# TMmichi/mujoco_jaco

Hardware: AMD Instinct MI355X
Metric: env-steps/sec at batch 65 536 (full Jaco + gripper + contacts) (higher is better)
Workload: dtype f32

## Files before the change

### mujoco_jaco_amd/csrc/collision.h

```cpp
#pragma once

#define JACO_HAVE_COLLISION 1

struct GeomPose { v3 p; m3 R; };
template <class L>
JDEV GeomPose geom_pose(const L& s, int g) { GeomPose r; r.p = ld3(s.gpos[g]); r.R = ldm(s.gmat[g]); return r; }

JDEV bool obb_separated(const GeomPose& a, v3 sa, const GeomPose& b, v3 sb) {
  float C[3][3], Q[3][3];
  v3 d = b.p - a.p;
  float t[3] = {dot(d, col(a.R, 0)), dot(d, col(a.R, 1)), dot(d, col(a.R, 2))};
  float ea[3] = {sa.x, sa.y, sa.z}, eb[3] = {sb.x, sb.y, sb.z};
#pragma unroll
  for (int i = 0; i < 3; i++)
#pragma unroll
    for (int j = 0; j < 3; j++) { C[i][j] = dot(col(a.R, i), col(b.R, j)); Q[i][j] = fabsf(C[i][j]) + 1e-5f; }
  bool sep = false;
#pragma unroll
  for (int i = 0; i < 3; i++) sep |= fabsf(t[i]) > ea[i] + eb[0] * Q[i][0] + eb[1] * Q[i][1] + eb[2] * Q[i][2];
#pragma unroll
  for (int j = 0; j < 3; j++)
    sep |= fabsf(t[0] * C[0][j] + t[1] * C[1][j] + t[2] * C[2][j]) > eb[j] + ea[0] * Q[0][j] + ea[1] * Q[1][j] + ea[2] * Q[2][j];
#pragma unroll
  for (int i = 0; i < 3; i++)
// ... 36 lines not shown
JDEV v3 support_geom(const JacoStepArgs& A, const JacoModelDev* m, const L& s, int g, int type, v3 dir, int lane) {
  GeomPose P = geom_pose(s, g);
  v3 l = mulT(P.R, dir), sp;
  if (type == JG_BOX) {
    sp = mk3(l.x > 0.f ? m->g_size[g][0] : -m->g_size[g][0], l.y > 0.f ? m->g_size[g][1] : -m->g_size[g][1], l.z > 0.f ? m->g_size[g][2] : -m->g_size[g][2]);
  } else if (type == JG_SPHERE) {
    float n = norm(l);
    sp = l * (n > JMINVAL ? m->g_size[g][0] / n : 0.f);
  } else {
    int adr = m->g_vertadr[g], nvert = m->g_vertnum[g];
    float best = -3.0e38f;
    int bi = 0x7fffffff;
    for (int i = lane; i < nvert; i += 64) {
      const float* v = A.hull + 4 * (size_t)(adr + i);
      float t = v[0] * l.x + v[1] * l.y + v[2] * l.z;
      if (t > best) { best = t; bi = i; }
    }
    float bv;
    int win = wave_argmax(best, bi, &bv);
    win = win < nvert ? win : 0;
    const float* v = A.hull + 4 * (size_t)(adr + win);
    sp = mk3(v[0], v[1], v[2]);
  }
  return P.p + mul(P.R, sp);
}

template <class L>
JDEV void collide_plane_box(v3 size, L& s, int g1, int g2, int pair, int lane, int& ncon, unsigned& flags) {
  GeomPose P = geom_pose(s, g1), B = geom_pose(s, g2);
  v3 n = col(P.R, 2);
  int i = lane & 7;
  v3 l = mk3((i & 1) ? size.x : -size.x, (i & 2) ? size.y : -size.y, (i & 4) ? size.z : -size.z);
  v3 c = B.p + mul(B.R, l);
  float dist = dot(c - P.p, n);
  push_contacts(s, lane < 8 && !(dist > 0.f), dist, c - n * (0.5f * dist), n, pair, ncon, flags, 4);
}
template <class L>
JDEV void collide_plane_sphere(const JacoModelDev* m, L& s, int g1, int g2, int pair, int lane, int& ncon, unsigned& flags) {
  GeomPose P = geom_pose(s, g1);
  v3 n = col(P.R, 2), c = ld3(s.gpos[g2]);
  float r = m->g_size[g2][0], dist = dot(c - P.p, n) - r;
  push_contacts(s, lane == 0 && !(dist > 0.f), dist, c - n * (r + 0.5f * dist), n, pair, ncon, flags, 1);
}
template <class L>
JDEV void collide_plane_convex(const JacoStepArgs& A, const JacoModelDev* m, L& s, int g1, int g2, int t2, int pair, int lane, int& ncon, unsigned& flags) {
  GeomPose P = geom_pose(s, g1);
  v3 n = col(P.R, 2);
  v3 sp = support_geom(A, m, s, g2, t2, -n, lane);
  float dist = dot(sp - P.p, n);
  push_contacts(s, lane == 0 && !(dist > 0.f), dist, sp - n * (0.5f * dist), n, pair, ncon, flags, 1);
}

template <class L>
JDEV void collide_box_box4(const JacoModelDev* m, L& s, int cbase, int nrows, int pkA, int codeA, unsigned m1A, unsigned m2A, int obA, int dimA,
                           v3 saA, v3 sbA, int lane, int& ncon, unsigned& flags) {
  constexpr int MAXCON = L::Caps::MAXCON;
  const int g = lane >> 4, a = lane & 15, rb = lane & 48;
  const bool slot = g < nrows;
  const int src = cbase + (slot ? g : 0);
  const int code = wave_shfl_i(codeA, src), pair = wave_shfl_i(pkA, src);
  const unsigned pm1 = (unsigned)wave_shfl_i((int)m1A, src), pm2 = (unsigned)wave_shfl_i((int)m2A, src);
  const int pob = wave_shfl_i(obA, src), pdim = wave_shfl_i(dimA, src);
  const int g1 = code & 255, g2 = (code >> 8) & 255;
  GeomPose P1 = geom_pose(s, g1), P2 = geom_pose(s, g2);
  float s1[3] = {wave_shfl(saA.x, src), wave_shfl(saA.y, src), wave_shfl(saA.z, src)}, s2[3] = {wave_shfl(sbA.x, src), wave_shfl(sbA.y, src), wave_shfl(sbA.z, src)};
  (void)m;
  v3 Aa[3] = {col(P1.R, 0), col(P1.R, 1), col(P1.R, 2)}, Ba[3] = {col(P2.R, 0), col(P2.R, 1), col(P2.R, 2)};
  v3 pp = P2.p - P1.p;
  const int ai = a < 15 ? a : 0;
  int ei = ai >= 6 ? (ai - 6) / 3 : (ai < 3 ? ai : 0), ej = ai >= 6 ? (ai - 6) % 3 : (ai >= 3 ? ai - 3 : 0);
  v3 Ai = ei == 0 ? Aa[0] : (ei == 1 ? Aa[1] : Aa[2]), Bj = ej == 0 ? Ba[0] : (ej == 1 ? Ba[1] : Ba[2]);
  v3 ax = ai < 3 ? Ai : (ai < 6 ? Bj : cross(Ai, Bj));
  float len = norm(ax);
  bool degenerate = ai >= 6 && len < 1e-6f;
  ax = ax * (1.f / fmaxf(len, 1e-30f));
  float ra = s1[0] * fabsf(dot(ax, Aa[0])) + s1[1] * fabsf(dot(ax, Aa[1])) + s1[2] * fabsf(dot(ax, Aa[2]));
  float rb_ = s2[0] * fabsf(dot(ax, Ba[0])) + s2[1] * fabsf(dot(ax, Ba[1])) + s2[2] * fabsf(dot(ax, Ba[2]));
  float dp = dot(pp, ax), pen = ra + rb_ - fabsf(dp);
  bool mine = slot && a < 15 && !degenerate;
  const unsigned long long sepm = wave_ballot(mine && pen < 0.f);
  const bool alive = slot && ((sepm >> rb) & 0xffffull) == 0ull;
  if (wave_ballot(alive) == 0ull) return;
  float fbest, ebest;
  int fcode = row_argmax(a < 6 ? -pen : -3.0e38f, a, &fbest);
  int ecode = row_argmax((a >= 6 && mine) ? -pen : -3.0e38f, a, &ebest);
  fbest = -fbest; ebest = -ebest;
  const bool edge = ebest < 1.0e38f && ebest * 1.05f < fbest;
  bool h1 = false, h2 = false;
  float d1 = 0.f, d2 = 0.f;
  v3 x1 = mk3(0, 0, 0), x2 = mk3(0, 0, 0), nrm = mk3(0, 0, 1.f);
  if (wave_ballot(alive && edge)) {
    const int ec = edge ? ecode : 6;
    const int i = (ec - 6) / 3, j = (ec - 6) % 3;
    float sgn = wave_shfl(dp, rb + ec) < 0.f ? -1.f : 1.f;
    v3 n = mk3(wave_shfl(ax.x, rb + ec), wave_shfl(ax.y, rb + ec), wave_shfl(ax.z, rb + ec)) * sgn;
    v3 ea = P1.p, eb = P2.p;
#pragma unroll
    for (int k = 0; k < 3; k++) {
      const v3 ea2 = ea + Aa[k] * (dot(n, Aa[k]) > 0.f ? s1[k] : -s1[k]), eb2 = eb + Ba[k] * (dot(n, Ba[k]) > 0.f ? -s2[k] : s2[k]);
      if (k != i) ea = ea2;
      if (k != j) eb = eb2;
    }
    v3 ua = i == 0 ? Aa[0] : (i == 1 ? Aa[1] : Aa[2]), ub = j == 0 ? Ba[0] : (j == 1 ? Ba[1] : Ba[2]);
    v3 r = eb - ea;
    float uv = dot(ua, ub), du = dot(r, ua), dv = dot(r, ub), den = 1.f - uv * uv;
    float sa = den > 1e-12f ? (du - uv * dv) / den : 0.f, tb = den > 1e-12f ? (uv * du - dv) / den : 0.f;
    if (alive && edge) {
      h1 = a == 0; d1 = -ebest; nrm = n;
      x1 = ((ea + ua * sa) + (eb + ub * tb)) * 0.5f;
    }
  }
  if (wave_ballot(alive && !edge)) {
    bool refis1 = fcode < 3;
    int ia = refis1 ? fcode : fcode - 3;
// ... 34 lines not shown
      const float kx = (k == 1 || k == 2) ? 1.f : -1.f, ky = k >= 2 ? 1.f : -1.f;
      const v3 q0 = c2 + eu * kx + ev * ky;
      if (a < 4) {
        hv1 = fabsf(q0.x) <= a_ && fabsf(q0.y) <= b_;
        pt1 = q0;
      } else if (a < 8) {
        float det = eu.x * ev.y - eu.y * ev.x;
        if (fabsf(det) > 1e-14f) {
          float x = kx * a_ - c2.x, y = ky * b_ - c2.y;
          float al = (x * ev.y - y * ev.x) / det, be = (eu.x * y - eu.y * x) / det;
          hv1 = fabsf(al) < 1.f && fabsf(be) < 1.f;
          pt1 = mk3(kx * a_, ky * b_, c2.z + al * eu.z + be * ev.z);
        }
      }
    }
    {
      const int k = a >> 2, k1 = (k + 1) & 3;
      const float kx = (k == 1 || k == 2) ? 1.f : -1.f, ky = k >= 2 ? 1.f : -1.f;
      const float k1x = (k1 == 1 || k1 == 2) ? 1.f : -1.f, k1y = k1 >= 2 ? 1.f : -1.f;
      const v3 q0 = c2 + eu * kx + ev * ky, q1 = c2 + eu * k1x + ev * k1y;
      const int e = a & 3, axn = e & 1;
      float lim = ((e & 2) ? 1.f : -1.f) * (axn ? b_ : a_), other = axn ? a_ : b_;
      float q0a = axn ? q0.y : q0.x, q1a = axn ? q1.y : q1.x, q0o = axn ? q0.x : q0.y, q1o = axn ? q1.x : q1.y;
      float e0 = q0a - lim, e1 = q1a - lim;
      if (!((e0 < 0.f) == (e1 < 0.f) || e0 == e1)) {
        float t = e0 / (e0 - e1);
        float o = q0o + t * (q1o - q0o);
        if (t > 0.f && t < 1.f && fabsf(o) < other) {
          hv2 = true;
          pt2 = axn ? mk3(o, lim, q0.z + t * (q1.z - q0.z)) : mk3(lim, o, q0.z + t * (q1.z - q0.z));
        }
      }
    }
    if (alive && !edge) {
      h1 = hv1 && !(pt1.z > 0.f); h2 = hv2 && !(pt2.z > 0.f);
      d1 = 0.5f * pt1.z; d2 = 0.5f * pt2.z;
      x1 = rp + Ru * pt1.x + Rv * pt1.y + nref * (rn + 0.5f * pt1.z);
      x2 = rp + Ru * pt2.x + Rv * pt2.y + nref * (rn + 0.5f * pt2.z);
      nrm = nref * (refis1 ? 1.f : -1.f);
    }
  }
  const unsigned long long M1 = wave_ballot(h1), M2 = wave_ballot(h2);
  int off = 0, tot = 0;
#pragma unroll
  for (int r = 0; r < 4; r++) {
    const int cr = popc64((M1 >> (16 * r)) & 0xffffull) + popc64((M2 >> (16 * r)) & 0xffffull);
    off += r < g ? cr : 0;
    tot += cr;
  }
  const unsigned long long r1 = (M1 >> rb) & 0xffffull, r2 = (M2 >> rb) & 0xffffull, below = (1ull << a) - 1ull;
  const int i1 = ncon + off + popc64(r1 & below), i2 = ncon + off + popc64(r1) + popc64(r2 & below);
  if (h1 && i1 < MAXCON) {
    s.c_dist[i1] = d1; st3(s.c_pos[i1], x1); make_frame(nrm, s.c_frame[i1]); s.c_pair[i1] = pair;
    s.c_m1[i1] = pm1; s.c_m2[i1] = pm2; s.c_ob[i1] = pob; s.c_dim[i1] = pdim;
  }
  if (h2 && i2 < MAXCON) {
    s.c_dist[i2] = d2; st3(s.c_pos[i2], x2); make_frame(nrm, s.c_frame[i2]); s.c_pair[i2] = pair;
    s.c_m1[i2] = pm1; s.c_m2[i2] = pm2; s.c_ob[i2] = pob; s.c_dim[i2] = pdim;
  }
  if (ncon + tot > MAXCON) { flags |= JFLAG_CON_OVERFLOW; tot = MAXCON - ncon; }
  ncon += tot;
}

struct Sup { v3 v, v1; };
struct MprGeom { GeomPose P; v3 size; int type, adr, nvert, cellR, celladr; };
#ifdef JACO_ROW_REUSE
struct HullRow { int cell; v4 e; };
#define JROWARG , HullRow& H1, HullRow& H2
#define JROWPASS , H1, H2
#else
#define JROWARG
#define JROWPASS
#endif
template <class L>
JDEV MprGeom mpr_geom(const JacoModelDev* m, const L& s, int g, int type) {
  MprGeom G;
  G.P = geom_pose(s, g);
  G.size = ld3(m->g_size[g]);
  G.type = type;
  G.adr = type == JG_MESH ? m->g_vertadr[g] : 0;
  G.nvert = type == JG_MESH ? m->g_vertnum[g] : 0;
  G.cellR = type == JG_MESH ? m->g_cellR[g] : 0;
  G.celladr = type == JG_MESH ? m->g_celladr[g] : 0;
  return G;
}
JDEV int cube_cell(v3 d, int R) {
  float ax = fabsf(d.x), ay = fabsf(d.y), az = fabsf(d.z);
  const bool fx = ax >= ay && ax >= az, fy = !fx && ay >= az;
  int face = fx ? (d.x > 0.f ? 0 : 1) : (fy ? (d.y > 0.f ? 2 : 3) : (d.z > 0.f ? 4 : 5));
  float mx = fx ? ax : (fy ? ay : az);
  mx = mx < 1e-30f ? 1.f : mx;
  float u = (fx ? d.y : d.x) / mx, v = ((fx || fy) ? d.z : d.y) / mx;
  int iu = (int)floorf((u + 1.f) * 0.5f * (float)R), iv = (int)floorf((v + 1.f) * 0.5f * (float)R);
  iu = iu < 0 ? 0 : (iu > R - 1 ? R - 1 : iu);
  iv = iv < 0 ? 0 : (iv > R - 1 ? R - 1 : iv);
  return (face * R + iu) * R + iv;
}
JDEV v3 support_prim(const MprGeom& G, v3 l) {
  if (G.type == JG_BOX) return mk3(l.x > 0.f ? G.size.x : -G.size.x, l.y > 0.f ? G.size.y : -G.size.y, l.z > 0.f ? G.size.z : -G.size.z);
  if (G.type == JG_CYLINDER) {
    const float rr = sqrtf(l.x * l.x + l.y * l.y), k = rr > JMINVAL ? G.size.x / rr : 0.f;
    return mk3(l.x * k, l.y * k, l.z > 0.f ? G.size.y : -G.size.y);
  }
  float n = norm(l);
  return l * (n > JMINVAL ? G.size.x / n : 0.f);
}
JDEV Sup mpr_support(const JacoStepArgs& A, const MprGeom& G1, const MprGeom& G2, v3 dir, int lane JROWARG) {
#ifdef JACO_EMULATED
  if (lane == 0) emu_counter[7]++;
#endif
  const v3 l1 = mulT(G1.P.R, dir), l2 = mulT(G2.P.R, -dir);
// ... 468 lines not shown
    for (int G = 0; 256 * G < npair; G++) {
      if (4 * G < plane_chunks) sphere_group<true>(s, m, G, npair, lane, n1, nl, tmp, PL::NV * 64); else sphere_group<false>(s, m, G, npair, lane, n1, nl, tmp, PL::NV * 64);
    }
#endif
    wave_sync();
    pl.n = nl <= PL::NV * 64 ? nl : -1;
    pl.planes = 0u;
#pragma unroll
    for (int j = 0; j < PL::NV; j++) {
      const bool have = j * 64 + lane < nl && pl.n >= 0;
      pl.e[j] = have ? tmp[have ? j * 64 + lane : 0] : 0u;
      pl.planes |= wave_ballot(have && ((pl.e[j] >> (JPL_KBITS + 2 * JPL_GBITS)) & 1u) != 0u) ? 1u << j : 0u;
    }
#pragma unroll
    for (int p = 0; p < JGEOM_PASSES; p++) { pl.px[p] = gp[p].x; pl.py[p] = gp[p].y; pl.pz[p] = gp[p].z; }
  } else {
#pragma unroll
    for (int j = 0; j < PL::NV; j++) {
      if (j * 64 < pl.n) {
        const bool valid = j * 64 + lane < pl.n;
        if ((pl.planes >> j) & 1u) list_chunk<true>(s, pl.e[j], valid, n1); else list_chunk<false>(s, pl.e[j], valid, n1);
      }
    }
  }
  JSTAMP(9);
  if (lane == 0) s.nsphere = n1;
  if (n1 > L::Caps::MAXCAND) { flags |= JFLAG_CAND_OVERFLOW; n1 = L::Caps::MAXCAND; }
  wave_sync();
  int ncand = 0;
  for (int base = 0; base < n1; base += 64) {
    int ci = base + lane;
    int k = ci < n1 ? s.cand[ci] : 0;
    bool keep = ci < n1;
    if (keep) {
      const v4 q0 = ld4(reinterpret_cast<const float*>(&m->pair_obb[k])), q1 = ld4(reinterpret_cast<const float*>(&m->pair_obb[k]) + 4);
      const int code = __builtin_bit_cast(int, q0.x);
      int g1 = code & 255, g2 = (code >> 8) & 255, t1 = (code >> 16) & 15;
      if (t1 != JG_PLANE) keep = !obb_separated(geom_pose(s, g1), mk3(q0.y, q0.z, q0.w), geom_pose(s, g2), mk3(q1.x, q1.y, q1.z));
    }
    wave_sync();
    unsigned long long mask = wave_ballot(keep);
    if (keep) s.cand[ncand + wave_prefix_count(mask)] = k;
    ncand += popc64(mask);
    wave_sync();
  }
  JSTAMP(10);
  int ncon = 0;
  for (int cb = 0; cb < ncand; cb += 64) {
    const int nhere = ncand - cb < 64 ? ncand - cb : 64;
    const int pkA = s.cand[lane < nhere ? cb + lane : cb];
    const v4 rec0 = ld4(reinterpret_cast<const float*>(&m->pair_obb[pkA])), rec1 = ld4(reinterpret_cast<const float*>(&m->pair_obb[pkA]) + 4);
    const int codeA = __builtin_bit_cast(int, rec0.x);
    const v3 saA = mk3(rec0.y, rec0.z, rec0.w), sbA = mk3(rec1.x, rec1.y, rec1.z);
    const unsigned m1A = m->pair[pkA].m1, m2A = m->pair[pkA].m2;
    const int obA = m->pair[pkA].ob, dimA = m->pair[pkA].condim;
    const unsigned long long boxes = wave_ballot(lane < nhere && ((codeA >> 16) & 255) == (JG_BOX | (JG_BOX << 4)));
    const unsigned long long hullc = wave_ballot(lane < nhere && ((codeA >> 16) & 15) != JG_PLANE && ((codeA >> 16) & 255) != (JG_BOX | (JG_BOX << 4)));
    v4 sepA; sepA.x = sepA.y = sepA.z = sepA.w = 0.f;
    float* const seprow = A.sepdir ? A.sepdir + (size_t)env * (4 * JMAXPAIR) : nullptr;
    if (seprow && lane < nhere && ((codeA >> 16) & 15) != JG_PLANE && ((codeA >> 16) & 255) != (JG_BOX | (JG_BOX << 4))) sepA = ld4(seprow + 4 * pkA);
    JSTAMP_NARROW(11);
#if JACO_MPR_PAIRS
    float* const stash = s.early_scratch;
    static_assert(JSCRATCH >= 512, "MPR result stash");
    unsigned long long parked = 0ull;
    if (A.mpr_pairs && popc64(hullc) >= 2) {
      const int gA1 = codeA & 255, gA2 = (codeA >> 8) & 255;
      const bool okA = lane < nhere && !((((codeA >> 16) & 15) == JG_MESH && m->g_cellR[gA1] == 0) || (((codeA >> 20) & 15) == JG_MESH && m->g_cellR[gA2] == 0));
      unsigned long long todo = hullc & wave_ballot(okA);
      while (popc64(todo) >= 2) {
        lane = wave_opaque_i(lane);
        const int c1 = ffs64(todo); todo &= todo - 1ull;
        const int c2 = ffs64(todo); todo &= todo - 1ull;
        const int cc = lane < 32 ? c1 : c2;
        const int pk2 = wave_shfl_i(pkA, cc), code2 = wave_shfl_i(codeA, cc);
        const MprGeom H1 = mpr_geom(m, s, code2 & 255, (code2 >> 16) & 15), H2 = mpr_geom(m, s, (code2 >> 8) & 255, (code2 >> 20) & 15);
        v4 sd; sd.x = wave_shfl(sepA.x, cc); sd.y = wave_shfl(sepA.y, cc); sd.z = wave_shfl(sepA.z, cc); sd.w = wave_shfl(sepA.w, cc);
        bool hit2, sv2, ran2;
        float depth2;
        v3 dir2, pos2, sep2;
        mpr_pair2(A, m, H1, H2, sd, true, lane, &hit2, &depth2, &dir2, &pos2, &sep2, &sv2, &ran2);
        if ((lane & 31) == 0) {
          if (seprow && ran2 && (sv2 || sd.w != 0.f)) {
            v4 o; o.x = sep2.x; o.y = sep2.y; o.z = sep2.z; o.w = sv2 ? 1.f : 0.f;
            *reinterpret_cast<v4*>(seprow + 4 * pk2) = o;
          }
          float* st = stash + 8 * cc;
          st[0] = hit2 ? 1.f : 0.f; st[1] = depth2; st[2] = pos2.x; st[3] = pos2.y; st[4] = pos2.z; st[5] = dir2.x; st[6] = dir2.y; st[7] = dir2.z;
#ifdef JACO_EMULATED
          emu_counter[3]++; emu_counter[4] += hit2;
#endif
        }
#ifdef JACO_EMULATED
        if (lane == 0) emu_counter[10]++;
#endif
        parked |= (1ull << c1) | (1ull << c2);
      }
      wave_sync();
      JSTAMP_NARROW(14);
    }
#else
    const unsigned long long parked = 0ull;
    (void)hullc;
#endif
    for (int c = 0; c < nhere;) {
      lane = wave_opaque_i(lane);
      if (L::Caps::MAXEFC < JacoHuge::MAXEFC && (wave_uniform_i((int)flags) & (int)JFLAG_CON_OVERFLOW)) break;
      if ((boxes >> c) & 1ull) {
        const int run = ffs64(~(boxes >> c) | 16ull);
        collide_box_box4(m, s, c, run, pkA, codeA, m1A, m2A, obA, dimA, saA, sbA, lane, ncon, flags);
        c += run;
        JSTAMP_NARROW(12);
        continue;
      }
      const int pk = wave_bcast_i(pkA, c), code = wave_bcast_i(codeA, c);
      const unsigned pm1 = (unsigned)wave_bcast_i((int)m1A, c), pm2 = (unsigned)wave_bcast_i((int)m2A, c);
      const int pob = wave_bcast_i(obA, c), pdim = wave_bcast_i(dimA, c);
      const int g1 = code & 255, g2 = (code >> 8) & 255, t1 = (code >> 16) & 15, t2 = (code >> 20) & 15;
      const int before = ncon;
      if (t1 == JG_PLANE) {
        if (t2 == JG_BOX) collide_plane_box(mk3(wave_bcast(sbA.x, c), wave_bcast(sbA.y, c), wave_bcast(sbA.z, c)), s, g1, g2, pk, lane, ncon, flags);
        else if (t2 == JG_SPHERE) collide_plane_sphere(m, s, g1, g2, pk, lane, ncon, flags);
        else if (t2 == JG_MESH) collide_plane_convex(A, m, s, g1, g2, t2, pk, lane, ncon, flags);
        JSTAMP_NARROW(13);
      } else {
        float depth;
        v3 dir, pos;
#ifdef JACO_EMULATED
        const long q0_ = emu_counter[7];
#endif
        const MprGeom G1 = mpr_geom(m, s, g1, t1), G2 = mpr_geom(m, s, g2, t2);
#ifdef JACO_ROW_REUSE
        HullRow H1, H2;
        H1.cell = -1; H2.cell = -1; H1.e.x = H1.e.y = H1.e.z = H1.e.w = 0.f; H2.e = H1.e;
#endif
        const float sw = wave_bcast(sepA.w, c);
        bool hit = false, apart = false, sepvalid = false;
        v3 sep = mk3(0.f, 0.f, 0.f);
#if JACO_MPR_PAIRS
        if ((parked >> c) & 1ull) {
          const float* st = stash + 8 * c;
          hit = st[0] != 0.f; depth = st[1]; pos = mk3(st[2], st[3], st[4]); dir = mk3(st[5], st[6], st[7]);
          apart = true;
        } else
#endif
        if (sw != 0.f) {
          const v3 d = mk3(wave_bcast(sepA.x, c), wave_bcast(sepA.y, c), wave_bcast(sepA.z, c));
          const Sup q = mpr_support(A, G1, G2, d, lane JROWPASS);
          apart = dot(q.v, d) < -1e-5f && fabsf(dot(d, d) - 1.f) < 1e-3f;
        }
        if (!apart) {
          hit = mpr_penetration(A, m, G1, G2, lane, &depth, &dir, &pos, &sep, &sepvalid JROWPASS);
          if (seprow && lane == 0 && (sepvalid || sw != 0.f)) {
            v4 o; o.x = sep.x; o.y = sep.y; o.z = sep.z; o.w = sepvalid ? 1.f : 0.f;
            *reinterpret_cast<v4*>(seprow + 4 * pk) = o;
          }
        }
#ifdef JACO_EMULATED
        if (lane == 0 && !((parked >> c) & 1ull)) { emu_counter[3]++; emu_counter[4] += hit; emu_counter[hit ? 5 : 6] += emu_counter[7] - q0_; }
#endif
#ifdef JACO_TRACE_MPR
        if (lane == 0) printf("mpr g1 %d g2 %d hit %d depth %g\n", g1, g2, (int)hit, hit ? depth : 0.f);
#endif
        push_contacts(s, hit && lane == 0, -depth, pos, dir, pk, ncon, flags, 1);
        JSTAMP_NARROW(hit ? 14 : 1);
      }
      if (ncon > before) {
        int cc = before + lane;
        if (cc < ncon) { s.c_m1[cc] = pm1; s.c_m2[cc] = pm2; s.c_ob[cc] = pob; s.c_dim[cc] = pdim; }
      }
      c++;
    }
    if (L::Caps::MAXEFC < JacoHuge::MAXEFC && (wave_uniform_i((int)flags) & (int)JFLAG_CON_OVERFLOW)) break;
  }
  if (lane == 0) { s.ncon = ncon; s.ncand = ncand; }
}

#define JSIDE_ROWS 16
#define JSIDE_BASE 64
#define JSIDE_J 0
#define JSIDE_AREF 96
#define JSIDE_D 112
#define JSIDE_F 128
template <class L>
struct SideRows {
  static constexpr bool on = L::Caps::CONTACT && L::Caps::MAXEFC == 64 && JNV - JB1 == 6 && (JNV - 6) * 6 + JNB * 6 >= JSIDE_F + JSIDE_ROWS;
};
template <class L>
JDEV float* side_buf(L& s) { return &s.cdof[6][0]; }
template <class L>
JDEV float contact_row_vel(const L& s, int c, int e, float mu) {
  const int pd = s.c_dim[c];
  const int kf = pd == 1 ? 0 : 1 + (e >> 1);
  const int obs = s.c_ob[c], b1 = ((obs >> 8) & 0xFF) - 1, b2 = ((obs >> 24) & 0xFF) - 1;
  sv v1, v2;
  v1.a = v1.b = v2.a = v2.b = mk3(0.f, 0.f, 0.f);
  if (b1 >= 0) v1 = ldsv(s.cvel[b1]);
  if (b2 >= 0) v2 = ldsv(s.cvel[b2]);
  v3 cp = ld3(s.c_pos[c]);
  v3 dw = v2.a - v1.a, dv = (v2.b - v1.b) + cross(dw, cp);
  const float* fr = s.c_frame[c];
  float vel = dot(ld3(fr), dv);
  if (pd > 1) {
    const int ax = kf < 3 ? kf : kf - 3;
    const float comp = dot(ld3(fr + 3 * ax), kf < 3 ? dv : dw);
    vel += ((e & 1) ? -1.f : 1.f) * mu * comp;
  }
  return vel;
}
template <class L>
JDEV void stage_contact_rows(const JacoModelDev* m, L& s, int lane, unsigned& flags) {
  constexpr int MAXEFC = L::Caps::MAXEFC;
  constexpr bool SIDE = SideRows<L>::on;
  const int nv = m->nv, ncon = wave_uniform_i(s.ncon), nlim = wave_uniform_i(s.nlimit);
  float* pa0 = reinterpret_cast<float*>(s.c_m1);
  float* pbc = reinterpret_cast<float*>(s.c_m2);
  float* sd = side_buf(s);
  int rowbase = nlim, kept_total = 0, nside = 0, side_cand = 0;
  constexpr int CPP = JNV <= 21 ? 3 : 64 / JNV;
  const int cl = lane / JNV, k = lane - cl * JNV;
  const bool dofok = cl < CPP && k < nv;
  const sv S = ldsv(s.cdof[dofok ? k : 0]);
  for (int cb = 0; cb < ncon; cb += 64) {
    const int ci = cb + lane, nhere = ncon - cb < 64 ? ncon - cb : 64;
    int dim = 0, nrow = 0;
    float mu0 = 0.f, mu1 = 0.f, mu2 = 0.f;
    unsigned cm1 = 0, cm2 = 0;
    float a0 = 0.f, bcoef = 0.f, dinv = 0.f;
    if (lane < nhere) {
      const JacoPairParam& P = m->pair[s.c_pair[ci]];
      dim = s.c_dim[ci]; nrow = dim == 1 ? 1 : 2 * (dim - 1);
      mu0 = P.mu[0]; mu1 = P.mu[2]; mu2 = P.mu[3];
      cm1 = s.c_m1[ci]; cm2 = s.c_m2[ci];
      const float pos = s.c_dist[ci] - P.margin, tran = P.tran;
      float R, imp;
      a0 = row_params(P.solref, P.solimp, pos, 0.f, dim == 1 ? tran : tran + mu0 * mu0 * tran, &R, &imp);
      bcoef = 2.f / fmaxf(JMINVAL, fminf(0.9999f, fmaxf(0.0001f, P.solimp[1])) * P.solref[0]);
      if (dim > 1) R = fmaxf(JMINVAL, 2.f * mu0 * mu0 * R);
      dinv = 1.f / R;
    }
    const unsigned mm = cm1 | cm2;
    bool sidec = false;
    const unsigned long long upto = lane >= 63 ? ~0ull : ((2ull << lane) - 1ull);
    const unsigned long long r1m = wave_ballot(nrow == 1), r4m = wave_ballot(nrow == 4), r10m = wave_ballot(nrow == 10);
    const bool rows_std = wave_ballot(nrow != 0 && nrow != 1 && nrow != 4 && nrow != 10) == 0ull;
    int end = rowbase + (rows_std ? popc64(r1m & upto) + 4 * popc64(r4m & upto) + 10 * popc64(r10m & upto) : wave_scan_incl(nrow, lane));
#ifdef JACO_SIDE_ALWAYS
    if (JNV - JB1 == 6 && cb == 0) {
#else
    if (JNV - JB1 == 6 && cb == 0 && wave_bcast_i(end, nhere - 1) > JSIDE_BASE) {
#endif
      const bool only2 = lane < nhere && mm != 0u && (mm & ((1u << JB1) - 1u)) == 0u && nrow <= 4;
      const bool reach2 = lane < nhere && !only2 && (mm >> JB1) != 0u;
      const unsigned long long o2 = wave_ballot(only2);
      if (o2 != 0ull && wave_ballot(reach2) == 0ull && ncon <= 64) {
        int srows = 0;
        for (unsigned long long b = o2; b; b &= b - 1ull) srows += wave_bcast_i(nrow, ffs64(b));
        if (srows <= JSIDE_ROWS) { side_cand = srows; sidec = only2; }
      }
    }
    bool split = false;
    int r0s = 0;
#ifdef JACO_SIDE_ALWAYS
    if (SIDE && side_cand > 0 && wave_bcast_i(end, nhere - 1) - side_cand <= MAXEFC) {
#else
    if (SIDE && side_cand > 0 && wave_bcast_i(end, nhere - 1) > MAXEFC && wave_bcast_i(end, nhere - 1) - side_cand <= MAXEFC) {
#endif
      split = true;
      end = rowbase + wave_scan_incl(sidec ? 0 : nrow, lane);
      r0s = JSIDE_BASE + wave_scan_incl(sidec ? nrow : 0, lane) - nrow;
      nside = side_cand;
    }
    sidec = sidec && split;
    const unsigned long long fm = wave_ballot(lane < nhere && end <= MAXEFC);
    const int kept = popc64(fm);
    int total = wave_bcast_i(end, kept > 0 ? kept - 1 : 0);
    total = kept > 0 ? total : rowbase;
    const int r0 = sidec ? r0s : end - nrow;
    if (lane < kept) {
      s.c_efc[ci] = r0;
      int blk = ((mm & ((1u << JB0) - 1u)) ? 1 : 0) | (((mm >> JB0) & ((1u << (JB1 - JB0)) - 1u)) ? 2 : 0) | ((mm >> JB1) ? 4 : 0);
      const int bodies = L::Caps::WRENCH ? ((((s.c_ob[ci] >> 8) & 31) << 19) | (((s.c_ob[ci] >> 24) & 31) << 24)) : 0;
      if (!sidec) for (int e = 0; e < nrow; e++) {
        s.e_con[r0 + e] = ci | (e << 8) | (blk << 16) | bodies;
        s.e_f[r0 + e] = e < 4 ? mu0 : (e < 6 ? mu1 : mu2);
      }
      pa0[ci] = a0; pbc[ci] = bcoef; s.c_fn[ci] = dinv;
    }
    wave_sync();
    for (int rr = rowbase + lane; rr < total; rr += 64) {
      const int ce = s.e_con[rr], c = ce & 255, e = (ce >> 8) & 255;
      const float vel = contact_row_vel(s, c, e, s.e_f[rr]);
      s.e_aref[rr] = pa0[c] - pbc[c] * vel;
      s.e_D[rr] = s.c_fn[c];
    }
    float aside[4] = {0.f, 0.f, 0.f, 0.f};
    if (SIDE && sidec && lane < kept) {
#pragma unroll
      for (int e = 0; e < 4; e++) if (e < nrow) aside[e] = a0 - bcoef * contact_row_vel(s, ci, e, mu0);
    }
    if (SIDE && split) {
      wave_sync();
      if (sidec && lane < kept) {
#pragma unroll
        for (int e = 0; e < 4; e++) if (e < nrow) { sd[JSIDE_AREF + r0 - JSIDE_BASE + e] = aside[e]; sd[JSIDE_D + r0 - JSIDE_BASE + e] = dinv; }
      }
    }
    if (L::Caps::WRENCH) {
      for (int rr = rowbase + lane; rr < total; rr += 64) {
        const int ce = s.e_con[rr], c = ce & 255, e = (ce >> 8) & 15, pd = s.c_dim[c];
        const int kf = pd == 1 ? 0 : 1 + (e >> 1);
        const float smu = ((e & 1) ? -1.f : 1.f) * s.e_f[rr];
        const float* fr = s.c_frame[c];
        const v3 n = ld3(fr), pos = ld3(s.c_pos[c]);
        v3 lin = n, ang = mk3(0.f, 0.f, 0.f);
        if (kf == 1 || kf == 2) lin = n + ld3(fr + 3 * kf) * smu;
        if (kf >= 3) ang = ld3(fr + 3 * (kf - 3)) * smu;
        ang = ang + cross(pos, lin);
        float* R = s.J + 8 * rr;
        R[0] = ang.x; R[1] = ang.y; R[2] = ang.z; R[3] = lin.x; R[4] = lin.y; R[5] = lin.z; R[6] = 0.f; R[7] = 0.f;
      }
    } else
    for (int c0 = 0; c0 < kept; c0 += CPP) {
      int c = c0 + (cl < CPP ? cl : 0);
      int src = c < 64 ? c : 0;
      int cdim = wave_shfl_i(dim, src), cr0 = wave_shfl_i(r0, src);
      float f0 = wave_shfl(mu0, src), f1 = wave_shfl(mu1, src), f2 = wave_shfl(mu2, src);
      unsigned a1 = (unsigned)wave_shfl_i((int)cm1, src), a2 = (unsigned)wave_shfl_i((int)cm2, src);
      const bool cside = SIDE && cr0 >= JSIDE_BASE;
      if (dofok && c < kept && (!cside || k >= JB1)) {
        float coef = (float)((int)((a2 >> k) & 1u) - (int)((a1 >> k) & 1u));
        v3 pos = ld3(s.c_pos[cb + c]);
        v3 jp = (S.b + cross(S.a, pos)) * coef, jr = S.a * coef;
        const float* fr = s.c_frame[cb + c];
        float Jc[6];
#pragma unroll
        for (int a = 0; a < 3; a++) { Jc[a] = dot(ld3(fr + 3 * a), jp); Jc[3 + a] = dot(ld3(fr + 3 * a), jr); }
        const int ld = cside ? 6 : JLD;
        float* Jw = cside ? sd + JSIDE_J + (cr0 - JSIDE_BASE) * 6 + (k - JB1) : s.J + cr0 * JLD + k;
        if (cdim == 1) Jw[0] = Jc[0];
        else {
          Jw[0] = Jc[0] + f0 * Jc[1]; Jw[ld] = Jc[0] - f0 * Jc[1];
          Jw[2 * ld] = Jc[0] + f0 * Jc[2]; Jw[3 * ld] = Jc[0] - f0 * Jc[2];
          if (cdim > 3) {
            Jw[4 * ld] = Jc[0] + f1 * Jc[3]; Jw[5 * ld] = Jc[0] - f1 * Jc[3];
            Jw[6 * ld] = Jc[0] + f2 * Jc[4]; Jw[7 * ld] = Jc[0] - f2 * Jc[4];
            Jw[8 * ld] = Jc[0] + f2 * Jc[5]; Jw[9 * ld] = Jc[0] - f2 * Jc[5];
// ... 99 lines not shown
```

### mujoco_jaco_amd/csrc/physics_kernel.h

```cpp
#pragma once
#include <stdint.h>
#include <jaco/model_dev.h>
#include <jaco/wave_ops.h>

#ifndef JACO_WRENCH
#define JACO_WRENCH 0
#endif
template <int MAXEFC_, int MAXCON_, int MAXCAND_, bool CONTACT_ = true>
struct JacoCaps {
  static_assert(MAXEFC_ % 64 == 0, "rows are dealt out 64 at a time (one per lane): the row capacity must be a multiple of 64");
  static constexpr bool WRENCH = CONTACT_ && JACO_WRENCH != 0;
  static_assert(WRENCH || JMAXGEOM != 64 || JNV != 21 || MAXCAND_ <= MAXEFC_ * 25 - 520 - 256 - 576, "default layout: the candidate list must fit behind the geom poses in the constraint-row area");
  static constexpr int MAXEFC = MAXEFC_, MAXCON = MAXCON_, MAXCAND = MAXCAND_, NR = MAXEFC_ / 64;
  static constexpr bool CONTACT = CONTACT_;
  static constexpr int JROWS = CONTACT_ ? MAXEFC_ : (JNB <= 16 ? 16 : 32), NGEOM = CONTACT_ ? JMAXGEOM : 1;
  static_assert(CONTACT_ || JNB <= 32, "limit rows of the contact-free instantiation");
};
#if JACO_WRENCH
typedef JacoCaps<128, 32, 240> JacoLight;
#else
typedef JacoCaps<64, 32, 240> JacoLight;
#endif
typedef JacoCaps<128, 32, 512> JacoMedium;
#ifndef JACO_HEAVY_ROWS
// ... 139 lines not shown
  return (const JacoStepArgs*)p;
}
#endif

#define JDBG_XPOS 0
#define JDBG_XMAT (JDBG_XPOS + 3 * JNB)
#define JDBG_M (JDBG_XMAT + 9 * JNB)
#define JDBG_BIAS (JDBG_M + JNV * JNV)
#define JDBG_SMOOTH (JDBG_BIAS + 24)
#define JDBG_QACC_SMOOTH (JDBG_SMOOTH + 24)
#define JDBG_QACC (JDBG_QACC_SMOOTH + 24)
#define JDBG_QFRC_CON (JDBG_QACC + 24)
#define JDBG_NCON (JDBG_QFRC_CON + 24)
#define JDBG_CONTACT (JDBG_NCON + 4)
#define JDBG_EFC (JDBG_CONTACT + 8 * JDBG_MAXCON)
#define JDBG_GPOS (JDBG_EFC + 4 * JDBG_MAXEFC)
#define JDBG_CFN (JDBG_GPOS + 3 * JMAXGEOM)
#define JDBG_SENS (JDBG_CFN + JDBG_MAXCON)
#define JDBG_SIZE (JDBG_SENS + JNSENS)

#define JMBLK (JB0 * JB0 + (JB1 - JB0) * (JB1 - JB0) + (JNV - JB1) * (JNV - JB1))
JDEV int m_index(int d, int j) {
  return d < JB0 ? d * JB0 + j : (d < JB1 ? JB0 * JB0 + (d - JB0) * (JB1 - JB0) + (j - JB0) : JB0 * JB0 + (JB1 - JB0) * (JB1 - JB0) + (d - JB1) * (JNV - JB1) + (j - JB1));
}
#define JTB_OFF (12 * JNV > 256 ? 12 * JNV : 256)
#define JSCRATCH (JTB_OFF + 16 * (JNB + 2) > 520 ? JTB_OFF + 16 * (JNB + 2) : 520)
#define JQ_LDS (JNQ + 1 > 24 ? JNQ + 1 : 24)
#define JV_LDS (JNV + 3 > 24 ? JNV + 3 : 24)
#define JU_LDS (JNU + 3 > 12 ? JNU + 3 : 12)
#define JFRAME_PASSES ((4 * (JNB + 2) + 63) / 64)
#define JGEOM_PASSES (JMAXGEOM / 64)

template <bool W> struct JacoChainTab { unsigned b_chain[JNB]; };
template <> struct JacoChainTab<false> {};
template <class C>
struct JacoLDS {
  typedef C Caps;
  float qpos[JQ_LDS], qvel[JV_LDS], qacc_ws[JV_LDS], ctrl[JU_LDS];
  float qpos_lo[JQ_LDS], qvel_lo[JV_LDS];
  float xpos[JNB][3], xmat[JNB][9];
  float cdof[JNV][6];
  float cvel[JNB][6];
  float M[JMBLK];
  float bias[JV_LDS], smooth[72];
  float mk[24];
  union {
    struct {
      alignas(16) float cinert[JNB][10];
      float crb[JNB][10];
      float cacc[JNB][6], cfrc[JNB][6];
    };
    struct {
      float c_dist[C::MAXCON], c_pos[C::MAXCON][3], c_frame[C::MAXCON][9], c_fn[C::MAXCON];
      int c_pair[C::MAXCON], c_efc[C::MAXCON];
      unsigned c_m1[C::MAXCON], c_m2[C::MAXCON];
      int c_ob[C::MAXCON];
      int c_dim[C::MAXCON];
    };
  };
  union {
    struct {
      alignas(16) float J[C::WRENCH ? (8 * C::MAXEFC > JSCRATCH ? 8 * C::MAXEFC : JSCRATCH) : C::JROWS * JLD];
      float e_aref[C::MAXEFC], e_D[C::MAXEFC], e_f[C::MAXEFC];
      int e_con[C::MAXEFC];
    };
    struct {
      float early_scratch[JSCRATCH];
      alignas(16) float gpos[C::NGEOM][4];
      float gmat[C::NGEOM][9];
      int cand[C::MAXCAND];
    };
  };
  float e_x[(C::MAXEFC > 64 && !C::WRENCH) ? C::MAXEFC : 1];
  int ncon, nefc, ncand, nlimit, nsphere;
  int nside, nside_cand;
  float task[JTASK_FLOATS];
  float osc_qd[4];
  struct McTab : JacoChainTab<C::WRENCH> {
    float b_pos[JNB][3], b_mat[JNB][9], b_axis[JNB][3], b_com[JNB][3], b_qpos0[JNB];
    int b_jtype[JNB], b_qadr[JNB], b_dadr[JNB], b_parent[JNB];
    int inner_body[JMAXINNER];
    unsigned b_descmask[JNB];
    int b_anc[JNB][3];
    int d_body[JNV], d_parent[JNV];
    int q_dof[JNQ + 1];
  } mc;
};
static_assert((JB1 - JB0 == 6 || JB1 == JB0) && (JNV - JB1 == 6 || JNV == JB1) && JB0 >= 6 && JNV <= 31 && JNV - JB0 <= 15 && JNV <= 64,
              "dof blocks: the arm tree(s) of at least the six arm joints, then zero, one or two free bodies; dofs + the residual column fit the 32-column matrix-core tile");

template <class L>
JDEV void stage_model(const JacoModelDev* m, L& s, int lane) {
  if (lane < JNB) {
    int b = lane;
    for (int k = 0; k < 3; k++) { s.mc.b_pos[b][k] = m->b_pos[b][k]; s.mc.b_axis[b][k] = m->b_axis[b][k]; s.mc.b_com[b][k] = m->b_com[b][k]; }
    for (int k = 0; k < 9; k++) s.mc.b_mat[b][k] = m->b_mat[b][k];
    s.mc.b_qpos0[b] = m->b_qpos0[b]; s.mc.b_jtype[b] = m->b_jtype[b]; s.mc.b_qadr[b] = m->b_qadr[b]; s.mc.b_dadr[b] = m->b_dadr[b];
    int p1 = m->b_parent[b], p2 = p1 >= 0 ? m->b_parent[p1] : -1, p3 = p2 >= 0 ? m->b_parent[p2] : -1, p4 = p3 >= 0 ? m->b_parent[p3] : -1;
    s.mc.b_parent[b] = p1;
    s.mc.b_descmask[b] = m->b_descmask[b];
    if constexpr (L::Caps::WRENCH) s.mc.b_chain[b] = m->b_chainmask[b];
    if (b < JMAXINNER) s.mc.inner_body[b] = m->inner_body[b];
    s.mc.b_anc[b][0] = p1; s.mc.b_anc[b][1] = p2; s.mc.b_anc[b][2] = p4;
    const int qa = m->b_qadr[b], da = m->b_dadr[b];
    if (b < m->nbody) {
      if (m->b_jtype[b] == JJ_HINGE) s.mc.q_dof[qa] = da;
      else { for (int k = 0; k < 3; k++) s.mc.q_dof[qa + k] = da + k; for (int k = 3; k < 7; k++) s.mc.q_dof[qa + k] = -1; }
    }
  }
  if (lane < JNV) { s.mc.d_body[lane] = m->d_body[lane]; s.mc.d_parent[lane] = m->d_parent[lane]; }
}

struct v3 { float x, y, z; };
JDEV v3 mk3(float x, float y, float z) { v3 r; r.x = x; r.y = y; r.z = z; return r; }
JDEV v3 ld3(const float* p) { return mk3(p[0], p[1], p[2]); }
JDEV void st3(float* p, v3 a) { p[0] = a.x; p[1] = a.y; p[2] = a.z; }
struct alignas(16) v4 { float x, y, z, w; };
JDEV v4 ld4(const float* p) { return *reinterpret_cast<const v4*>(p); }
JDEV v3 operator+(v3 a, v3 b) { return mk3(a.x + b.x, a.y + b.y, a.z + b.z); }
JDEV v3 operator-(v3 a, v3 b) { return mk3(a.x - b.x, a.y - b.y, a.z - b.z); }
JDEV v3 operator*(v3 a, float s) { return mk3(a.x * s, a.y * s, a.z * s); }
JDEV v3 operator*(float s, v3 a) { return mk3(a.x * s, a.y * s, a.z * s); }
JDEV v3 operator-(v3 a) { return mk3(-a.x, -a.y, -a.z); }
JDEV float dot(v3 a, v3 b) { return a.x * b.x + a.y * b.y + a.z * b.z; }
JDEV v3 cross(v3 a, v3 b) { return mk3(a.y * b.z - a.z * b.y, a.z * b.x - a.x * b.z, a.x * b.y - a.y * b.x); }
JDEV float norm(v3 a) { return sqrtf(dot(a, a)); }
JDEV v3 normalized(v3 a) {
  float n = norm(a);
  return n < JMINVAL ? mk3(1.f, 0.f, 0.f) : a * (1.f / n);
}
struct m3 { float m[9]; };
JDEV m3 ldm(const float* p) { m3 r; for (int i = 0; i < 9; i++) r.m[i] = p[i]; return r; }
JDEV void stm(float* p, const m3& a) { for (int i = 0; i < 9; i++) p[i] = a.m[i]; }
JDEV v3 mul(const m3& a, v3 v) {
  return mk3(a.m[0] * v.x + a.m[1] * v.y + a.m[2] * v.z, a.m[3] * v.x + a.m[4] * v.y + a.m[5] * v.z, a.m[6] * v.x + a.m[7] * v.y + a.m[8] * v.z);
}
JDEV v3 mulT(const m3& a, v3 v) {
  return mk3(a.m[0] * v.x + a.m[3] * v.y + a.m[6] * v.z, a.m[1] * v.x + a.m[4] * v.y + a.m[7] * v.z, a.m[2] * v.x + a.m[5] * v.y + a.m[8] * v.z);
}
JDEV m3 mul(const m3& a, const m3& b) {
// ... 1870 lines not shown
    wave_sync();
    if (lane < JTASK_N) { if (wt) st_wt(&A.task[(size_t)env * JTASK_N + lane], s.task[lane]); else A.task[(size_t)env * JTASK_N + lane] = s.task[lane]; }
  }
  if (reset_now) {
    wave_sync();
    if (lane < nq) { s.qpos[lane] = A.qpos0[lane]; s.qpos_lo[lane] = 0.f; }
    if (lane < nv) { s.qvel[lane] = 0.f; s.qvel_lo[lane] = 0.f; s.qacc_ws[lane] = 0.f; }
    if (lane < nu) s.ctrl[lane] = 0.f;
    if (lane < 24) {
      const float r = m->marker_rest[lane / 12][lane % 12];
      s.mk[lane] = r;
      if (A.marker) st_wt(&A.marker[(size_t)env * 24 + lane], r);
    }
    wave_sync();
    if (lane == 0) {
      reset_draws(A.task_id, A.seed, (unsigned)env, nq >= 23, m->base_pos, s.qpos, s.task, GoalBuffer{A.goal_buf, A.goal_n, A.goal_stride});
      s.task[JT_FWD] = 1.f;
      if (A.hint) st_wt_i(&A.hint[env], 0);
    }
    wave_sync();
    fwd = true; sub0 = 0; nsub = 1; left = 0; calm = 0;
    goto again;
  }
  unsigned long long anyf = wave_ballot(flags != 0);
  if (anyf) {
    unsigned f = flags;
    for (int o = 1; o < 64; o <<= 1) f |= (unsigned)wave_shfl_i((int)f, lane ^ o);
    if (lane == 0 && A.flags) { if (bailed) or_wt(&A.flags[env], f); else A.flags[env] |= f; }
  }
  if (!LIGHT && left == 0 && nsub > 0 && lane == 0 && A.hint && A.hint_mode == 2) {
    const int nc = s.ncon, ne = s.nefc, ns = s.nsphere;
    const bool light_rows = ne <= JacoLight::MAXEFC || (SideRows<JacoLDS<JacoLight>>::on && s.nside_cand > 0 && ne - s.nside_cand <= JacoLight::MAXEFC);
    A.hint[env] = (nc <= JacoLight::MAXCON && light_rows && ns <= JacoLight::MAXCAND) ? 0
                : ((nc <= JacoMedium::MAXCON && ne <= JacoMedium::MAXEFC && ns <= JacoMedium::MAXCAND) ? 1
                : ((nc <= JacoHeavy::MAXCON && ne <= JacoHeavy::MAXEFC && ns <= JacoHeavy::MAXCAND) ? 2 : 3));
  }
  if (left == 0 && lane == 0 && A.stats) {
    A.stats[4 * env] = s.ncon; A.stats[4 * env + 1] = s.nefc + s.nside; A.stats[4 * env + 2] = iters; A.stats[4 * env + 3] = s.ncand | (nls_last << 16);
  }
  wave_sync();
  if (why) *why = left <= 0 ? 0 : (bailed ? 1 : 2);
  return left;
#undef A
}

#ifdef JACO_TU
#define JACO_TU_HAS(n) (JACO_TU == (n))
#else
#define JACO_TU_HAS(n) 1
#endif
#ifndef JACO_LIGHT_WAVES
#define JACO_LIGHT_WAVES 3
#endif
template <bool FULL, class C = JacoLight>
JDEV void light_grid(const JacoStepArgs& A, JacoLDS<C>& s) {
  const int lane = lane_id();
  if (env_id() >= A.nenv) return;
  const int nslots = A.nslots ? *A.nslots : A.nenv;
  for (int slot = env_id(); slot < nslots; slot += grid_size()) {
  const int env = A.order ? A.order[slot] : slot;
  if (A.routed_mark && A.routed_mark[env] == A.launch_id) return;
  const bool masked_out = FULL && JM_MASKED(A.env_mode) && A.mask && !A.mask[env];
  int left = 0;
  if (!masked_out) {
    if (FULL && A.hint && JM_MASKED(A.env_mode) && lane == 0) st_wt_i(&A.hint[env], 0);
    const unsigned long long t_start = wave_clock();
    left = run_env<C, 0, FULL>(A, s, env, A.nsub, lane);
    if (lane == 0 && A.cost && JM_REAL_STEP(A.env_mode)) { unsigned c = (unsigned)((wave_clock() - t_start) >> 4); if (left > 0) st_wt_u(&A.cost[env], c); else A.cost[env] = c; }
    if (left > 0) queue_push(A, (FULL && A.env_mode == JM_FORWARD) ? 2 : 0, env, left, lane);
  }
  wave_sync();
  }
  if (lane == 0 && A.light_left) jaco_atomic_dec(A.light_left, false);
}
#if JACO_TU_HAS(0)
__global__ __launch_bounds__(64, JACO_LIGHT_WAVES) void jaco_physics_kernel(JacoStepArgs A) {
  __shared__ JacoLDS<JacoLight> s;
  JEMU_POISON(s);
  light_grid<false>(A, s);
}
#endif
#if JACO_TU_HAS(1)
__global__ __launch_bounds__(64, JACO_LIGHT_WAVES) void jaco_physics_kernel_listed(JacoStepArgs A) {
  __shared__ JacoLDS<JacoLight> s;
  JEMU_POISON(s);
  light_grid<true>(A, s);
}
#endif
#if JACO_TU_HAS(8)
__global__ __launch_bounds__(64, 4) void jaco_physics_kernel_arm(JacoStepArgs A) {
  __shared__ JacoLDS<JacoArm> s;
  JEMU_POISON(s);
  light_grid<false, JacoArm>(A, s);
}
#endif
template <class BIG, int TB, class U>
JDEV int run_env_tiers(const JacoStepArgs& A, U& u, int env, int lane) {
  const unsigned long long t_start = wave_clock();
  const bool stepmode = JM_TASK_SUBSTEPS(A.env_mode);
  int left = stepmode ? A.nsub : A.remaining[env], why = 0;
  for (;;) {
    left = run_env<BIG, TB>(A, u.big, env, stepmode ? A.nsub : left, lane, !A.no_tier_return, &why);
    if (left <= 0 || why == 1) break;
    wave_sync();
    left = run_env<JacoLight, 0>(A, u.light, env, stepmode ? A.nsub : left, lane);
    if (left <= 0) break;
// ... 193 lines not shown
```

Before: 1.903 million.

## Shrink per-env LDS footprint so more light-tier envs fit per CU

Drops the per-contact m1/m2 arrays from LDS and reads them from the pair parameters at constraint build time. Index arrays for pairs, dims, bodies and dofs are narrowed to 16-bit and 8-bit types. The per-contact a0/dinv values are written straight into the e_aref/e_D rows instead of staging buffers. A static_assert checks that the light tier's LDS, rounded to allocation granules, fits 4×JACO_LIGHT_WAVES envs per CU, which allows higher occupancy. In exchange it adds sub-word LDS accesses and an extra global read of the pair parameters.

```diff
diff --git a/mujoco_jaco_amd/csrc/collision.h b/mujoco_jaco_amd/csrc/collision.h
--- a/mujoco_jaco_amd/csrc/collision.h
+++ b/mujoco_jaco_amd/csrc/collision.h
@@ -112,14 +112,13 @@
 }
 
 template <class L>
-JDEV void collide_box_box4(const JacoModelDev* m, L& s, int cbase, int nrows, int pkA, int codeA, unsigned m1A, unsigned m2A, int obA, int dimA,
+JDEV void collide_box_box4(const JacoModelDev* m, L& s, int cbase, int nrows, int pkA, int codeA, int obA, int dimA,
                            v3 saA, v3 sbA, int lane, int& ncon, unsigned& flags) {
   constexpr int MAXCON = L::Caps::MAXCON;
   const int g = lane >> 4, a = lane & 15, rb = lane & 48;
   const bool slot = g < nrows;
   const int src = cbase + (slot ? g : 0);
   const int code = wave_shfl_i(codeA, src), pair = wave_shfl_i(pkA, src);
-  const unsigned pm1 = (unsigned)wave_shfl_i((int)m1A, src), pm2 = (unsigned)wave_shfl_i((int)m2A, src);
   const int pob = wave_shfl_i(obA, src), pdim = wave_shfl_i(dimA, src);
   const int g1 = code & 255, g2 = (code >> 8) & 255;
   GeomPose P1 = geom_pose(s, g1), P2 = geom_pose(s, g2);
@@ -260,11 +259,11 @@
   const int i1 = ncon + off + popc64(r1 & below), i2 = ncon + off + popc64(r1) + popc64(r2 & below);
   if (h1 && i1 < MAXCON) {
     s.c_dist[i1] = d1; st3(s.c_pos[i1], x1); make_frame(nrm, s.c_frame[i1]); s.c_pair[i1] = pair;
-    s.c_m1[i1] = pm1; s.c_m2[i1] = pm2; s.c_ob[i1] = pob; s.c_dim[i1] = pdim;
+    s.c_ob[i1] = pob; s.c_dim[i1] = pdim;
   }
   if (h2 && i2 < MAXCON) {
     s.c_dist[i2] = d2; st3(s.c_pos[i2], x2); make_frame(nrm, s.c_frame[i2]); s.c_pair[i2] = pair;
-    s.c_m1[i2] = pm1; s.c_m2[i2] = pm2; s.c_ob[i2] = pob; s.c_dim[i2] = pdim;
+    s.c_ob[i2] = pob; s.c_dim[i2] = pdim;
   }
   if (ncon + tot > MAXCON) { flags |= JFLAG_CON_OVERFLOW; tot = MAXCON - ncon; }
   ncon += tot;
@@ -839,7 +838,6 @@
     const v4 rec0 = ld4(reinterpret_cast<const float*>(&m->pair_obb[pkA])), rec1 = ld4(reinterpret_cast<const float*>(&m->pair_obb[pkA]) + 4);
     const int codeA = __builtin_bit_cast(int, rec0.x);
     const v3 saA = mk3(rec0.y, rec0.z, rec0.w), sbA = mk3(rec1.x, rec1.y, rec1.z);
-    const unsigned m1A = m->pair[pkA].m1, m2A = m->pair[pkA].m2;
     const int obA = m->pair[pkA].ob, dimA = m->pair[pkA].condim;
     const unsigned long long boxes = wave_ballot(lane < nhere && ((codeA >> 16) & 255) == (JG_BOX | (JG_BOX << 4)));
     const unsigned long long hullc = wave_ballot(lane < nhere && ((codeA >> 16) & 15) != JG_PLANE && ((codeA >> 16) & 255) != (JG_BOX | (JG_BOX << 4)));
@@ -895,13 +893,12 @@
       if (L::Caps::MAXEFC < JacoHuge::MAXEFC && (wave_uniform_i((int)flags) & (int)JFLAG_CON_OVERFLOW)) break;
       if ((boxes >> c) & 1ull) {
         const int run = ffs64(~(boxes >> c) | 16ull);
-        collide_box_box4(m, s, c, run, pkA, codeA, m1A, m2A, obA, dimA, saA, sbA, lane, ncon, flags);
+        collide_box_box4(m, s, c, run, pkA, codeA, obA, dimA, saA, sbA, lane, ncon, flags);
         c += run;
         JSTAMP_NARROW(12);
         continue;
       }
       const int pk = wave_bcast_i(pkA, c), code = wave_bcast_i(codeA, c);
-      const unsigned pm1 = (unsigned)wave_bcast_i((int)m1A, c), pm2 = (unsigned)wave_bcast_i((int)m2A, c);
       const int pob = wave_bcast_i(obA, c), pdim = wave_bcast_i(dimA, c);
       const int g1 = code & 255, g2 = (code >> 8) & 255, t1 = (code >> 16) & 15, t2 = (code >> 20) & 15;
       const int before = ncon;
@@ -954,7 +951,7 @@
       }
       if (ncon > before) {
         int cc = before + lane;
-        if (cc < ncon) { s.c_m1[cc] = pm1; s.c_m2[cc] = pm2; s.c_ob[cc] = pob; s.c_dim[cc] = pdim; }
+        if (cc < ncon) { s.c_ob[cc] = pob; s.c_dim[cc] = pdim; }
       }
       c++;
     }
@@ -1000,8 +997,6 @@
   constexpr int MAXEFC = L::Caps::MAXEFC;
   constexpr bool SIDE = SideRows<L>::on;
   const int nv = m->nv, ncon = wave_uniform_i(s.ncon), nlim = wave_uniform_i(s.nlimit);
-  float* pa0 = reinterpret_cast<float*>(s.c_m1);
-  float* pbc = reinterpret_cast<float*>(s.c_m2);
   float* sd = side_buf(s);
   int rowbase = nlim, kept_total = 0, nside = 0, side_cand = 0;
   constexpr int CPP = JNV <= 21 ? 3 : 64 / JNV;
@@ -1018,7 +1013,7 @@
       const JacoPairParam& P = m->pair[s.c_pair[ci]];
       dim = s.c_dim[ci]; nrow = dim == 1 ? 1 : 2 * (dim - 1);
       mu0 = P.mu[0]; mu1 = P.mu[2]; mu2 = P.mu[3];
-      cm1 = s.c_m1[ci]; cm2 = s.c_m2[ci];
+      cm1 = P.m1; cm2 = P.m2;
       const float pos = s.c_dist[ci] - P.margin, tran = P.tran;
       float R, imp;
       a0 = row_params(P.solref, P.solimp, pos, 0.f, dim == 1 ? tran : tran + mu0 * mu0 * tran, &R, &imp);
@@ -1071,15 +1066,15 @@
       if (!sidec) for (int e = 0; e < nrow; e++) {
         s.e_con[r0 + e] = ci | (e << 8) | (blk << 16) | bodies;
         s.e_f[r0 + e] = e < 4 ? mu0 : (e < 6 ? mu1 : mu2);
-      }
-      pa0[ci] = a0; pbc[ci] = bcoef; s.c_fn[ci] = dinv;
+        s.e_aref[r0 + e] = a0; s.e_D[r0 + e] = dinv;
+      }
+      s.c_fn[ci] = bcoef;
     }
     wave_sync();
     for (int rr = rowbase + lane; rr < total; rr += 64) {
       const int ce = s.e_con[rr], c = ce & 255, e = (ce >> 8) & 255;
       const float vel = contact_row_vel(s, c, e, s.e_f[rr]);
-      s.e_aref[rr] = pa0[c] - pbc[c] * vel;
-      s.e_D[rr] = s.c_fn[c];
+      s.e_aref[rr] = s.e_aref[rr] - s.c_fn[c] * vel;
     }
     float aside[4] = {0.f, 0.f, 0.f, 0.f};
     if (SIDE && sidec && lane < kept) {
diff --git a/mujoco_jaco_amd/csrc/physics_kernel.h b/mujoco_jaco_amd/csrc/physics_kernel.h
--- a/mujoco_jaco_amd/csrc/physics_kernel.h
+++ b/mujoco_jaco_amd/csrc/physics_kernel.h
@@ -215,10 +215,9 @@
     };
     struct {
       float c_dist[C::MAXCON], c_pos[C::MAXCON][3], c_frame[C::MAXCON][9], c_fn[C::MAXCON];
-      int c_pair[C::MAXCON], c_efc[C::MAXCON];
-      unsigned c_m1[C::MAXCON], c_m2[C::MAXCON];
       int c_ob[C::MAXCON];
-      int c_dim[C::MAXCON];
+      unsigned short c_pair[C::MAXCON], c_efc[C::MAXCON];
+      unsigned char c_dim[C::MAXCON];
     };
   };
   union {
@@ -241,14 +240,15 @@
   float osc_qd[4];
   struct McTab : JacoChainTab<C::WRENCH> {
     float b_pos[JNB][3], b_mat[JNB][9], b_axis[JNB][3], b_com[JNB][3], b_qpos0[JNB];
-    int b_jtype[JNB], b_qadr[JNB], b_dadr[JNB], b_parent[JNB];
     int inner_body[JMAXINNER];
     unsigned b_descmask[JNB];
-    int b_anc[JNB][3];
-    int d_body[JNV], d_parent[JNV];
-    int q_dof[JNQ + 1];
+    signed char b_jtype[JNB], b_qadr[JNB], b_dadr[JNB], b_parent[JNB];
+    signed char b_anc[JNB][3];
+    signed char d_body[JNV], d_parent[JNV];
+    signed char q_dof[JNQ + 1];
   } mc;
 };
+static_assert(JMAXPAIR <= 65536 && JNB <= 127 && JNQ <= 127, "sub-word index arrays of JacoLDS: pair indices in 16 bits, body / dof / coordinate indices in a signed byte");
 static_assert((JB1 - JB0 == 6 || JB1 == JB0) && (JNV - JB1 == 6 || JNV == JB1) && JB0 >= 6 && JNV <= 31 && JNV - JB0 <= 15 && JNV <= 64,
               "dof blocks: the arm tree(s) of at least the six arm joints, then zero, one or two free bodies; dofs + the residual column fit the 32-column matrix-core tile");
 
@@ -2225,6 +2225,12 @@
 #ifndef JACO_LIGHT_WAVES
 #define JACO_LIGHT_WAVES 3
 #endif
+#define JACO_LDS_GRANULE 1280
+#define JACO_LDS_PER_CU (160 * 1024)
+#if JNB == 11 && JNV == 21 && JMAXGEOM == 64 && !JACO_WRENCH
+static_assert((sizeof(JacoLDS<JacoLight>) + JACO_LDS_GRANULE - 1) / JACO_LDS_GRANULE * JACO_LDS_GRANULE * (4 * JACO_LIGHT_WAVES) <= JACO_LDS_PER_CU,
+              "default layout: the light tier's LDS, rounded up to whole allocation blocks, must fit 4 x JACO_LIGHT_WAVES envs per CU (<= 12 800 B)");
+#endif
 template <bool FULL, class C = JacoLight>
 JDEV void light_grid(const JacoStepArgs& A, JacoLDS<C>& s) {
   const int lane = lane_id();
```

Result: faster. 2.031 million (median of 6 runs) (+6.7%).
